# StellaOrg/ImplicitBVH.jl

Measured on AMD Instinct MI355X. Metric: BVH build+traverse throughput, higher is better.
Workload: dtype f32; 1 GPU; 1000000 random BSphere{Float32} leaves per GPU, BBox{Float32} nodes, UInt32 Morton, Int32 index, build + LVT self-traverse + read of the contact count (BASELINE.json configs[1]); leaves_per_gpu=1000000, leaves_total=1000000, contacts_total=1763579, parallelism=single GPU

## Files before the change

implicitbvh.jl_amd/csrc/ibvh_lvt_queue.inc:

```
#include "ibvh_lvt.hpp"

namespace ibvh {
namespace lvt {

#define IBVH_DPP_STEP(CTRL)                              \
    "v_min_f32_dpp %0, %0, %0 " CTRL "\n\t"              \
    "v_min_f32_dpp %1, %1, %1 " CTRL "\n\t"              \
    "v_min_f32_dpp %2, %2, %2 " CTRL "\n\t"              \
    "v_min_f32_dpp %3, %3, %3 " CTRL "\n\t"              \
    "v_min_f32_dpp %4, %4, %4 " CTRL "\n\t"              \
    "v_min_f32_dpp %5, %5, %5 " CTRL "\n\t"              \
    "v_max_f32_dpp %6, %6, %6 " CTRL "\n\t"              \
    "v_max_f32_dpp %7, %7, %7 " CTRL "\n\t"              \
    "v_max_f32_dpp %8, %8, %8 " CTRL "\n\t"              \
    "v_max_f32_dpp %9, %9, %9 " CTRL "\n\t"              \
    "v_max_f32_dpp %10, %10, %10 " CTRL "\n\t"           \
    "v_max_f32_dpp %11, %11, %11 " CTRL "\n\t"
IBVH_D void wave_prefix_scans_dpp(float (&mn)[6], float (&mx)[6]) {
    asm volatile("s_nop 1\n\t" IBVH_DPP_STEP("row_shr:1 row_mask:0xf bank_mask:0xf") IBVH_DPP_STEP("row_shr:2 row_mask:0xf bank_mask:0xf")
                     IBVH_DPP_STEP("row_shr:4 row_mask:0xf bank_mask:0xf") IBVH_DPP_STEP("row_shr:8 row_mask:0xf bank_mask:0xf")
                         IBVH_DPP_STEP("row_bcast:15 row_mask:0xa bank_mask:0xf") IBVH_DPP_STEP("row_bcast:31 row_mask:0xc bank_mask:0xf")
                 : "+v"(mn[0]), "+v"(mn[1]), "+v"(mn[2]), "+v"(mn[3]), "+v"(mn[4]), "+v"(mn[5]), "+v"(mx[0]), "+v"(mx[1]), "+v"(mx[2]),
                   "+v"(mx[3]), "+v"(mx[4]), "+v"(mx[5]));
}
#undef IBVH_DPP_STEP
IBVH_D float wave_min_dpp_lane63(float v) {
    asm volatile("s_nop 1\n\t"
                 "v_min_f32_dpp %0, %0, %0 row_shr:1 row_mask:0xf bank_mask:0xf\n\ts_nop 1\n\t"
                 "v_min_f32_dpp %0, %0, %0 row_shr:2 row_mask:0xf bank_mask:0xf\n\ts_nop 1\n\t"
                 "v_min_f32_dpp %0, %0, %0 row_shr:4 row_mask:0xf bank_mask:0xf\n\ts_nop 1\n\t"
                 "v_min_f32_dpp %0, %0, %0 row_shr:8 row_mask:0xf bank_mask:0xf\n\ts_nop 1\n\t"
                 "v_min_f32_dpp %0, %0, %0 row_bcast:15 row_mask:0xa bank_mask:0xf\n\ts_nop 1\n\t"
                 "v_min_f32_dpp %0, %0, %0 row_bcast:31 row_mask:0xc bank_mask:0xf\n\ts_nop 1"
                 : "+v"(v));
    return v;
}

#define IBVH_TEST_AND_APPEND(SFX, SEVENTH)                                                                                \
    asm volatile("s_mov_b64 exec, %[init]\n\t"                                                                           \
                 "v_cmpx_le" SFX " %[slo0], %[vup0]\n\t"                                                                 \
                 "v_cmpx_ge" SFX " %[sup0], %[vlo0]\n\t"                                                                 \
                 "v_cmpx_le" SFX " %[slo1], %[vup1]\n\t"                                                                 \
                 "v_cmpx_ge" SFX " %[sup1], %[vlo1]\n\t"                                                                 \
                 "v_cmpx_le" SFX " %[slo2], %[vup2]\n\t"                                                                 \
                 "v_cmpx_ge" SFX " %[sup2], %[vlo2]\n\t" SEVENTH "s_nop 2\n\t"                                          \
                 "v_mbcnt_lo_u32_b32 %[tmp], exec_lo, 0\n\t"                                                             \
                 "v_mbcnt_hi_u32_b32 %[tmp], exec_hi, %[tmp]\n\t"                                                        \
                 "v_lshl_add_u32 %[tmp], %[tmp], 2, %[addr]\n\t"                                                         \
                 "ds_write_b32 %[tmp], %[e]\n\t"                                                                         \
                 "s_bcnt1_i32_b64 %[cnt], exec\n\t"                                                                      \
                 "s_mov_b64 exec, -1\n\t"                                                                                \
                 "s_lshl2_add_u32 %[addr], %[cnt], %[addr]"                                                              \
                 : [tmp] "=&v"(tmp), [cnt] "=&s"(cnt), [addr] "+s"(lds_addr)                                             \
                 : [init] "s"(init), [slo0] "s"(slo0), [slo1] "s"(slo1), [slo2] "s"(slo2), [sup0] "s"(sup0), [sup1] "s"(sup1), \
                   [sup2] "s"(sup2), [vlo0] "v"(vlo0), [vlo1] "v"(vlo1), [vlo2] "v"(vlo2), [vup0] "v"(vup0), [vup1] "v"(vup1), \
                   [vup2] "v"(vup2), [sthr] "s"(sthr), [vcmp] "v"(vcmp), [e] "v"(e)                                      \
                 : "vcc", "scc", "memory")

#define IBVH_CONTACT_MASK(SFX)                                                                                                                \
    asm volatile("s_mov_b64 exec, %[init]\n\t"                                                                                               \
                 "v_cmpx_le" SFX " %[slo0], %[vup0]\n\t"                                                                                     \
                 "v_cmpx_ge" SFX " %[sup0], %[vlo0]\n\t"                                                                                     \
                 "v_cmpx_le" SFX " %[slo1], %[vup1]\n\t"                                                                                     \
                 "v_cmpx_ge" SFX " %[sup1], %[vlo1]\n\t"                                                                                     \
                 "v_cmpx_le" SFX " %[slo2], %[vup2]\n\t"                                                                                     \
                 "v_cmpx_ge" SFX " %[sup2], %[vlo2]\n\t"                                                                                     \
                 "s_mov_b64 %[m], exec\n\t"                                                                                                  \
                 "s_mov_b64 exec, -1"                                                                                                        \
                 : [m] "=&s"(m)                                                                                                              \
                 : [init] "s"(init), [slo0] "s"(S.lo[0]), [slo1] "s"(S.lo[1]), [slo2] "s"(S.lo[2]), [sup0] "s"(S.up[0]), [sup1] "s"(S.up[1]), \
                   [sup2] "s"(S.up[2]), [vlo0] "v"(V.lo[0]), [vlo1] "v"(V.lo[1]), [vlo2] "v"(V.lo[2]), [vup0] "v"(V.up[0]), [vup1] "v"(V.up[1]), \
                   [vup2] "v"(V.up[2])                                                                                                       \
                 : "vcc")

#define IBVH_CONTACT_MASK2(SFX)                                                                                                               \
    asm volatile("s_mov_b64 exec, %[init]\n\t"                                                                                               \
                 "v_cmpx_le" SFX " %[alo0], %[vup0]\n\t"                                                                                     \
                 "v_cmpx_ge" SFX " %[aup0], %[vlo0]\n\t"                                                                                     \
                 "v_cmpx_le" SFX " %[alo1], %[vup1]\n\t"                                                                                     \
                 "v_cmpx_ge" SFX " %[aup1], %[vlo1]\n\t"                                                                                     \
                 "v_cmpx_le" SFX " %[alo2], %[vup2]\n\t"                                                                                     \
                 "v_cmpx_ge" SFX " %[aup2], %[vlo2]\n\t"                                                                                     \
                 "s_mov_b64 %[ma], exec\n\t"                                                                                                 \
                 "s_mov_b64 exec, %[init]\n\t"                                                                                               \
                 "v_cmpx_le" SFX " %[blo0], %[vup0]\n\t"                                                                                     \
                 "v_cmpx_ge" SFX " %[bup0], %[vlo0]\n\t"                                                                                     \
                 "v_cmpx_le" SFX " %[blo1], %[vup1]\n\t"                                                                                     \
                 "v_cmpx_ge" SFX " %[bup1], %[vlo1]\n\t"                                                                                     \
                 "v_cmpx_le" SFX " %[blo2], %[vup2]\n\t"                                                                                     \
                 "v_cmpx_ge" SFX " %[bup2], %[vlo2]\n\t"                                                                                     \
                 "s_or_b64 %[m], %[ma], exec\n\t"                                                                                            \
                 "s_mov_b64 exec, -1"                                                                                                        \
                 : [m] "=&s"(m), [ma] "=&s"(ma)                                                                                              \
                 : [init] "s"(init), [alo0] "s"(A.lo[0]), [alo1] "s"(A.lo[1]), [alo2] "s"(A.lo[2]), [aup0] "s"(A.up[0]), [aup1] "s"(A.up[1]), \
                   [aup2] "s"(A.up[2]), [blo0] "s"(B.lo[0]), [blo1] "s"(B.lo[1]), [blo2] "s"(B.lo[2]), [bup0] "s"(B.up[0]), [bup1] "s"(B.up[1]), \
                   [bup2] "s"(B.up[2]), [vlo0] "v"(V.lo[0]), [vlo1] "v"(V.lo[1]), [vlo2] "v"(V.lo[2]), [vup0] "v"(V.up[0]), [vup1] "v"(V.up[1]), \
                   [vup2] "v"(V.up[2])                                                                                                       \
                 : "vcc", "scc")

#define IBVH_BOX_ASM(T, SFX)                                                                                                                  \
    template <bool THR_GE, bool PRUNE = true>                                                                                                \
    IBVH_D void test_and_append(uint64_t init, T slo0, T slo1, T slo2, T sup0, T sup1, T sup2, T vlo0, T vlo1, T vlo2, T vup0, T vup1, T vup2, \
                                uint32_t sthr, uint32_t vcmp, uint32_t e, uint32_t &lds_addr) {                                              \
        uint32_t tmp, cnt;                                                                                                                   \
        if constexpr (!PRUNE) IBVH_TEST_AND_APPEND(SFX, "");                                                                                 \
        else if constexpr (THR_GE) IBVH_TEST_AND_APPEND(SFX, "v_cmpx_ge_u32 %[sthr], %[vcmp]\n\t");                                          \
        else IBVH_TEST_AND_APPEND(SFX, "v_cmpx_lt_u32 %[sthr], %[vcmp]\n\t");                                                                \
    }                                                                                                                                        \
    IBVH_D uint64_t contact_mask(uint64_t init, const BBox<T> &S, const BBox<T> &V) {                                                        \
        uint64_t m;                                                                                                                          \
        IBVH_CONTACT_MASK(SFX);                                                                                                              \
        return m;                                                                                                                            \
    }                                                                                                                                        \
    IBVH_D uint64_t contact_mask2(uint64_t init, const BBox<T> &A, const BBox<T> &B, const BBox<T> &V) {                                     \
        uint64_t m, ma;                                                                                                                      \
        IBVH_CONTACT_MASK2(SFX);                                                                                                             \
        return m;                                                                                                                            \
    }
IBVH_BOX_ASM(float, "_f32")
IBVH_BOX_ASM(double, "_f64")
#undef IBVH_BOX_ASM
#undef IBVH_CONTACT_MASK2
#undef IBVH_CONTACT_MASK
#undef IBVH_TEST_AND_APPEND

IBVH_D void split_two_boxes_f32(const BBox<float> &mine, bool use, int lane, BBox<float> &ubox_a, BBox<float> &ubox_b) {
    using N = BBox<float>;
    const float big = float_max<float>();
    auto half_area = [](const N &b) {
        float d[3];
#pragma unroll
        for (int k = 0; k < 3; ++k) {
            d[k] = b.up[k] - b.lo[k];
            d[k] = d[k] > 0.0f ? d[k] : 0.0f;
        }
        return d[0] * d[1] + d[1] * d[2] + d[0] * d[2];
    };
    N pre, rev, rsuf;
#pragma unroll
    for (int k = 0; k < 3; ++k) {
        pre.lo[k] = use ? mine.lo[k] : big;
        pre.up[k] = use ? mine.up[k] : -big;
        rev.lo[k] = __shfl(pre.lo[k], 63 - lane, 64);
        rev.up[k] = __shfl(pre.up[k], 63 - lane, 64);
    }
    {
        float mn[6] = {pre.lo[0], pre.lo[1], pre.lo[2], rev.lo[0], rev.lo[1], rev.lo[2]};
        float mx[6] = {pre.up[0], pre.up[1], pre.up[2], rev.up[0], rev.up[1], rev.up[2]};
        wave_prefix_scans_dpp(mn, mx);
#pragma unroll
        for (int k = 0; k < 3; ++k) {
            pre.lo[k] = mn[k];
            pre.up[k] = mx[k];
            rsuf.lo[k] = mn[3 + k];
            rsuf.up[k] = mx[3 + k];
        }
    }
    const float ra = half_area(rsuf);
    float sa = __shfl(ra, 62 - lane, 64);
    sa = lane == 63 ? 0.0f : sa;
    float cost = half_area(pre) + sa;
    cost = cost == cost ? cost : __builtin_inff();
    const float m = wave_min_dpp_lane63(cost);
    const float best = __int_as_float(__builtin_amdgcn_readlane(__float_as_int(m), 63));
    const uint64_t at = __builtin_amdgcn_ballot_w64(cost == best);
    const int ksplit = at != 0 ? (int)__builtin_ctzll(at) : 0;
    ubox_a = broadcast_from_lane(pre, ksplit);
    ubox_b = broadcast_from_lane(rsuf, ksplit == 63 ? 0 : 62 - ksplit);
    if (ksplit == 63) {
#pragma unroll
        for (int k = 0; k < 3; ++k) {
            ubox_b.lo[k] = big;
            ubox_b.up[k] = -big;
        }
    }
}

template <class N> struct BlockFrontier {
    const N *nodes;
    TreeDev tree;
    const N *q_nodes;
    TreeDev q_tree;
    int32_t shift, start_level, cut_level, self;
    uint32_t *rows;
};
template <class N, bool PAIRED> __global__ __launch_bounds__(64) void lvt_block_frontier_kernel(BlockFrontier<N> f) {
    __shared__ uint32_t s_fr[2][BLK_FCAP];
    const int lane = threadIdx.x;
    const uint32_t b = blockIdx.x;
    uint32_t *row = f.rows + (size_t)b * BLK_ROW;
    const int levels = (int)f.tree.levels;
    const uint32_t vl = (uint32_t)f.tree.virtual_leaves;
    auto num_real = [&](int level) -> uint32_t { return (1u << (level - 1)) - (vl >> (levels - level)); };
    auto first_mem = [&](int level) -> uint32_t {
        const uint32_t v = vl >> (levels - (level - 1));
        return (1u << (level - 1)) - (2u * v - (uint32_t)__builtin_popcount(v)) - 1u;
    };
    const int qlevels = (int)f.q_tree.levels;
    const uint32_t qvl = (uint32_t)f.q_tree.virtual_leaves;
    const int blevel = qlevels - f.shift;
    const uint32_t qv = qvl >> (qlevels - (blevel - 1));
    const uint32_t q_first = (1u << (blevel - 1)) - (2u * qv - (uint32_t)__builtin_popcount(qv)) - 1u;
    const N bbox = load_vol_uniform<N>(f.q_nodes + (q_first + b));
    bool ok = true;
#pragma unroll
    for (int k = 0; k < 3; ++k) ok = ok && bbox.lo[k] == bbox.lo[k] && bbox.up[k] == bbox.up[k];
    if (lane == 0) *(N *)(row + 2) = bbox;
    if (!ok) {
        if (lane == 0) row[0] = 0xffffffffu;
        return;
    }
    const uint32_t block_next = (b << f.shift) + (1u << (levels - 1)) + 1u;
    const int start_level = f.start_level, cut_level = f.cut_level;
    auto touches = [&](const N &box, uint32_t idx, int lvl) {
        bool h = iscontact(bbox, box);
        if (f.self) h = h & !((idx + 1u) <= (block_next >> (levels - lvl)));
        return h;
    };
    int count = (int)num_real(start_level);
    for (int i = lane; i < count; i += 64) s_fr[0][i] = (1u << (start_level - 1)) + (uint32_t)i;
    __builtin_amdgcn_wave_barrier();
    uint32_t *cur = s_fr[0], *nxt = s_fr[1];
    const uint64_t lt_mask = ((uint64_t)1 << lane) - 1;
    int out = 0;
    bool overflow = false;
    int lvl = start_level;
    while (lvl <= cut_level && count > 0 && !overflow) {
        const N *lvl_nodes = f.nodes + first_mem(lvl);
        const uint32_t lvl_first = 1u << (lvl - 1);
        int next_count = 0;
        const bool paired = PAIRED && lvl < cut_level;
        if (paired) {
            const int cl = lvl + 1;
            const N *ch_nodes = f.nodes + first_mem(cl);
            const uint32_t ch_first = 1u << (cl - 1), ch_last = ch_first + num_real(cl) - 1u;
            const uint32_t gc_last = cl < levels ? (1u << cl) + num_real(cl + 1) - 1u : 0u;
            for (int base = 0; base < count; base += 64) {
                const bool have = base + lane < count;
                const uint32_t idx = cur[have ? base + lane : base];
                const uint32_t c0 = 2u * idx, c1 = c0 + 1u;
                const bool real1 = c1 <= ch_last;
                const N box = load_vol<N>(lvl_nodes + (idx - lvl_first));
                const N b0 = load_vol<N>(ch_nodes + (c0 - ch_first));
                const N b1 = load_vol<N>(ch_nodes + ((real1 ? c1 : c0) - ch_first));
                const bool hit = have & touches(box, idx, lvl);
                const bool h0 = hit & touches(b0, c0, cl), h1 = hit & real1 & touches(b1, c1, cl);
                const uint64_t m0 = __builtin_amdgcn_ballot_w64(h0), m1 = __builtin_amdgcn_ballot_w64(h1);
                const int before = __popcll(m0 & lt_mask) + __popcll(m1 & lt_mask), total = __popcll(m0) + __popcll(m1);
                if (cl == cut_level) {
                    if (out + total > BLK_CAP) {
                        overflow = true;
                        break;
                    }
                    if (h0) row[BLK_HEAD + out + before] = c0;
                    if (h1) row[BLK_HEAD + out + before + (h0 ? 1 : 0)] = c1;
                    out += total;
                } else {
                    if (next_count + 2 * total > BLK_FCAP) {
                        overflow = true;
                        break;
                    }
                    const int at = next_count + 2 * before;
                    if (h0) {
                        nxt[at] = 2u * c0;
                        nxt[at + 1] = 2u * c0 + 1u;
                    }
                    if (h1) {
                        nxt[at + (h0 ? 2 : 0)] = 2u * c1;
                        nxt[at + (h0 ? 2 : 0) + 1] = 2u * c1 + 1u;
                    }
                    const uint64_t any = m0 | m1;
                    bool last_virtual = false;
                    if (any != 0) {
                        const int top = 63 - __builtin_clzll(any);
                        const uint32_t ti = (uint32_t)__builtin_amdgcn_readlane((int)idx, top);
                        const uint32_t tc = ((m1 >> top) & 1u) ? 2u * ti + 1u : 2u * ti;
                        last_virtual = 2u * tc + 1u > gc_last;
                    }
                    next_count = __builtin_amdgcn_readfirstlane(next_count + 2 * total - (last_virtual ? 1 : 0));
                }
            }
            lvl += 2;
        } else {
            const uint32_t child_real = lvl < levels ? num_real(lvl + 1) : 0u;
            for (int base = 0; base < count; base += 64) {
                const bool have = base + lane < count;
                const uint32_t idx = cur[have ? base + lane : base];
                const N box = load_vol<N>(lvl_nodes + (idx - lvl_first));
                const bool hit = have & touches(box, idx, lvl);
                const uint64_t hm = __builtin_amdgcn_ballot_w64(hit);
                const int before = __popcll(hm & lt_mask), total = __popcll(hm);
                if (lvl == cut_level) {
                    if (out + total > BLK_CAP) {
                        overflow = true;
                        break;
                    }
                    if (hit) row[BLK_HEAD + out + before] = idx;
                    out += total;
                } else {
                    const bool last_virtual = hm != 0 && [&] {
                        const int top = 63 - __builtin_clzll(hm);
                        const uint32_t ti = (uint32_t)__builtin_amdgcn_readlane((int)idx, top);
                        return (2u * ti + 1u - (1u << lvl)) >= child_real;
                    }();
                    const int add = __builtin_amdgcn_readfirstlane(2 * total - (last_virtual ? 1 : 0));
                    if (next_count + add > BLK_FCAP) {
                        overflow = true;
                        break;
                    }
                    if (hit) {
                        nxt[next_count + 2 * before] = 2u * idx;
                        if (2 * before + 1 < add) nxt[next_count + 2 * before + 1] = 2u * idx + 1u;
                    }
                    next_count = __builtin_amdgcn_readfirstlane(next_count + add);
                }
            }
            lvl += 1;
        }
        __builtin_amdgcn_wave_barrier();
        uint32_t *t = cur;
        cur = nxt;
        nxt = t;
        count = __builtin_amdgcn_readfirstlane(lvl > cut_level ? 0 : next_count);
    }
    if (lane == 0) row[0] = overflow ? 0xffffffffu : (uint32_t)out;
}

#ifdef IBVH_PHASE_STAMPS
__device__ unsigned long long g_lvt_ticks[8];
struct Sections {
    unsigned long long t0, acc[6] = {0, 0, 0, 0, 0, 0};
    IBVH_D void start() { t0 = __builtin_amdgcn_s_memtime(); }
    IBVH_D void lap(int k) {
        const unsigned long long t = __builtin_amdgcn_s_memtime();
        acc[k] += t - t0;
        t0 = t;
    }
    IBVH_D void flush() {
        if ((threadIdx.x & 63) == 0) {
#pragma unroll
            for (int k = 0; k < 6; ++k) atomicAdd(&g_lvt_ticks[k], acc[k]);
            atomicAdd(&g_lvt_ticks[7], 1ull);
        }
    }
};
#else
struct Sections {
    IBVH_D void start() {}
    IBVH_D void lap(int) {}
    IBVH_D void flush() {}
};
#endif
enum { SEC_PROLOGUE = 0, SEC_DESCENT = 1, SEC_SUBTREE = 2, SEC_LOOPS = 3, SEC_LEAVES = 4, SEC_EPILOGUE = 5 };

constexpr int QUEUE_CAP = 512;
constexpr int QUEUE_WAVES = 1;
constexpr int QUEUE_MINWAVES = 7;

template <class L, class N, class I, bool WIDE, bool WRITE = false> constexpr int queue_min_waves() {
    if (sizeof(typename N::elt) == 8) return 4;
    if (sizeof(typename L::elt) == 8) return 5;
    if (WIDE && sizeof(I) == 8) return 6;
    return WRITE ? QUEUE_MINWAVES - 1 : QUEUE_MINWAVES;
}
template <class L, class N, class I, int MODE, bool WRITE, bool NARROW, bool WIDE, bool COUNT = false, class Q = L>
__global__ __launch_bounds__(64 * QUEUE_WAVES, (queue_min_waves<L, N, I, WIDE, WRITE>())) void lvt_queue_kernel(Args<L, N, I> a, PairCache<I> cache, int cut_level) {
    using TN = typename N::elt;
    static_assert(std::is_same<TN, float>::value || std::is_same<TN, double>::value,
                  "walker 2's box tests are assembly for Float32 and Float64 nodes (IBVH_BOX_ASM): a new node element type starts in dispatch_leaf_node");
    Work<COUNT> work;
    using QS = Query<L, N, I, MODE, WRITE, NARROW, Q>;
    using Cnt = typename QS::Cnt;
    __shared__ uint32_t s_frontier[QUEUE_WAVES][2][FRONTIER_CAP];
    using QE = typename std::conditional<WIDE, uint64_t, uint32_t>::type;
    __shared__ QE s_queue[QUEUE_WAVES][QUEUE_CAP];
    __shared__ Cnt s_cnt[QUEUE_WAVES][64];
    __shared__ I s_qside[QUEUE_WAVES][64];
    Sections sec;
    sec.start();
    const bool dense_index = WRITE && a.q_index_dense != nullptr;
    QS q(a, cache, dense_index);
    const int lane = threadIdx.x & 63, wv = __builtin_amdgcn_readfirstlane((int)(threadIdx.x >> 6));
    if constexpr (!WRITE && !COUNT) {
        if (a.q_index_dense != nullptr && q.valid) a.q_index_dense[q.item] = q.q_index;
        if (a.scan_agg != nullptr && lane == 0) {
            const int gw = (int)blockIdx.x * QUEUE_WAVES + wv;
            if (gw < a.scan_nparts) a.scan_agg[gw] = 0ull;
        }
    }
    struct Entry {
        I other;
        I meta;
    };
    const int64_t first_item = q.item - lane;
    const int64_t items_here = a.n_items - first_item < 64 ? a.n_items - first_item : 64;
    char *region = cache.K > 0 && items_here > 0 ? (char *)(cache.slots + first_item * (int64_t)cache.K) : nullptr;
    const int entry_cap = region ? (int)(((int64_t)items_here * cache.K * (int64_t)sizeof(IndexPair<I>) - 16) / (int64_t)sizeof(Entry)) : 0;
    Entry *entries = (Entry *)(region + 16);
    int wfill = 0;
    if constexpr (WRITE) {
        const int64_t guard = a.guard_total != nullptr ? load_total_uniform(a.guard_total) : 0;
        q.w = (q.valid && q.item > 0) ? (Cnt)a.counts[q.item - 1] : 0;
        const I q_side = a.positions ? (I)(q.item + 1) : ((dense_index && q.valid) ? a.q_index_dense[q.item] : q.q_index);
        const int fill_raw = region ? *(const int *)region : -1;
        constexpr bool SPECULATE = MODE == MODE_SELF;
        Entry e0 = {}, e1 = {};
        if constexpr (SPECULATE) {
            if (region && entry_cap > 0) {
                e0 = entries[lane < entry_cap ? lane : entry_cap - 1];
                e1 = entries[lane + 64 < entry_cap ? lane + 64 : entry_cap - 1];
            }
        }
        if (a.guard_total != nullptr && guard > a.guard_capacity) return;
        const int fill = __builtin_amdgcn_readfirstlane(fill_raw);
        if (fill >= 0) {
            s_cnt[wv][lane] = q.w;
            s_qside[wv][lane] = q_side;
            __builtin_amdgcn_wave_barrier();
            for (int t = lane; t < fill; t += 64) {
                const Entry e = !SPECULATE ? entries[t] : (t < 64 ? e0 : (t < 128 ? e1 : entries[t]));
                const int qi = (int)(e.meta & 63);
                const int64_t dest = (int64_t)s_cnt[wv][qi] + (int64_t)(e.meta >> 6);
                const I qv = s_qside[wv][qi];
                IndexPair<I> c2;
                if (a.positions) c2 = (MODE == MODE_PAIR && a.flip) ? IndexPair<I>{e.other, qv} : IndexPair<I>{qv, e.other};
                else if constexpr (MODE == MODE_SELF) c2 = qv > e.other ? IndexPair<I>{e.other, qv} : IndexPair<I>{qv, e.other};
                else c2 = a.flip ? IndexPair<I>{e.other, qv} : IndexPair<I>{qv, e.other};
                a.contacts[dest] = c2;
            }
            return;
        }
        if (dense_index) q.load_leaf();
        q.lane_on = q.valid;
    }
    if constexpr (MODE == MODE_PAIR) {
        if (a.built_level <= 1 && a.tree.levels >= 2) {
            const N root = load_vol_uniform<N>(a.nodes);
            work.add(0, q.lane_on);
            work.add(2, lane == 0);
            if (__builtin_amdgcn_ballot_w64(q.lane_on & iscontact(q.q_node, root)) == 0) {
                work.flush(a.work);
                if constexpr (!WRITE) {
                    if (q.valid) a.counts[q.item] = (I)0;
                    if (region && lane == 0) *(int *)region = 0;
                }
                return;
            }
        }
    }

    const int levels = (int)a.tree.levels;
    const uint32_t vl = (uint32_t)a.tree.virtual_leaves;
    auto num_real = [&](int level) -> uint32_t { return (1u << (level - 1)) - (vl >> (levels - level)); };
    auto first_mem = [&](int level) -> uint32_t {
        const uint32_t v = vl >> (levels - (level - 1));
        return (1u << (level - 1)) - (2u * v - (uint32_t)__builtin_popcount(v)) - 1u;
    };
    const uint32_t leaf_first = 1u << (levels - 1);
    const uint32_t my_item = (uint32_t)q.item;
    const uint32_t wave_item0 = (uint32_t)__builtin_amdgcn_readfirstlane((int)my_item);
    const uint32_t self_next = my_item + leaf_first + 1u;
    const uint32_t wave_next = wave_item0 + leaf_first + 1u;
    QE *queue = s_queue[wv];
    Cnt *cnts = s_cnt[wv];
    cnts[lane] = WRITE ? q.w : (Cnt)0;
    int qn = 0;
    const uint64_t lane_on_mask = __builtin_amdgcn_ballot_w64(q.lane_on);
    const uint32_t *blk_row = nullptr;
    int blk_count = -1;
    uint32_t blk_idx0 = 0;
    if constexpr (!COUNT) {
        if (a.blk_rows != nullptr) {
            blk_row = a.blk_rows + (size_t)(wave_item0 >> a.blk_shift) * BLK_ROW;
            blk_count = (int)*(const __attribute__((address_space(4))) uint32_t *)(uintptr_t)blk_row;
            blk_count = blk_count > BLK_CAP ? -1 : blk_count;
            blk_idx0 = blk_row[BLK_HEAD + lane];
        }
    }

    N ubox_a, ubox_b;
    {
        bool use = q.lane_on;
#pragma unroll
        for (int k = 0; k < 3; ++k) use = use && q.q_node.lo[k] == q.q_node.lo[k] && q.q_node.up[k] == q.q_node.up[k];
        if constexpr (std::is_same<TN, float>::value) {
            split_two_boxes_f32(q.q_node, use, lane, ubox_a, ubox_b);
        } else {
            BBox<float> qf, fa, fb;
#pragma unroll
            for (int k = 0; k < 3; ++k) {
                qf.lo[k] = __double2float_rd(q.q_node.lo[k]);
                qf.up[k] = __double2float_ru(q.q_node.up[k]);
            }
            split_two_boxes_f32(qf, use, lane, fa, fb);
#pragma unroll
            for (int k = 0; k < 3; ++k) {
                ubox_a.lo[k] = (double)fa.lo[k];
                ubox_a.up[k] = (double)fa.up[k];
                ubox_b.lo[k] = (double)fb.lo[k];
                ubox_b.up[k] = (double)fb.up[k];
            }
        }
    }
    bool use_rows = false;
    if constexpr (!COUNT) {
        if (blk_count >= 0) {
            const N bb = load_vol_uniform<N>(blk_row + 2);
            bool outside = false;
#pragma unroll
            for (int k = 0; k < 3; ++k) {
                const bool isnum = q.q_node.lo[k] == q.q_node.lo[k] && q.q_node.up[k] == q.q_node.up[k];
                outside = outside | (isnum & !(q.q_node.lo[k] >= bb.lo[k] && q.q_node.up[k] <= bb.up[k]));
            }
            bool allnum = true;
#pragma unroll
            for (int k = 0; k < 3; ++k) allnum = allnum && q.q_node.lo[k] == q.q_node.lo[k] && q.q_node.up[k] == q.q_node.up[k];
            use_rows = __builtin_amdgcn_ballot_w64(q.lane_on & allnum & outside) == 0;
        }
    }
    const int lp = levels - 1;
    const uint32_t lp_real = num_real(lp);
    const N *lp_nodes = a.nodes + first_mem(lp);
    const uint32_t n_leaves = (uint32_t)a.tree.real_leaves;
    const uint64_t lt_mask = ((uint64_t)1 << lane) - 1;

    auto pair_step = [&](int off, int avail) {
        const bool v = lane < avail;
        const QE e = queue[off + (v ? lane : 0)];
        const int qi = (int)(e & 63u);
        const uint32_t pos = 2u * (uint32_t)(e >> 6);
        const bool has_b = v & (pos + 1u < n_leaves);
        uint64_t mor_a = 0, mor_b = 0;
        const char *rec = a.leaves + (int64_t)pos * a.lay.stride;
        const char *rec_b = (pos + 1u < n_leaves) ? rec + a.lay.stride : rec;
        const L leaf_a = load_vol<L>(rec), leaf_b = load_vol<L>(rec_b);
        const I idx_a = load_index<I>(rec, a.lay), idx_b = load_index<I>(rec_b, a.lay);
        if constexpr (NARROW) {
            if (a.narrow == IBVH_NARROW_MORTON_LT) {
                mor_a = load_morton(rec, a.lay);
                mor_b = load_morton(rec_b, a.lay);
            }
        }
        const Q ql = shuffle_from(q.q_leaf, qi);
        const I qidx = __shfl(q.q_index, qi, 64);
        const uint32_t item_q = wave_item0 + (uint32_t)qi;
        bool hit_a = v & iscontact(ql, leaf_a), hit_b = has_b & iscontact(ql, leaf_b);
        work.add(1, (uint32_t)v + (uint32_t)has_b);
        work.add(3, (uint32_t)v + (uint32_t)has_b);
        if constexpr (MODE == MODE_SELF) {
            hit_a = hit_a & (pos > item_q);
            hit_b = hit_b & (pos + 1u > item_q);
        }
        if constexpr (NARROW) {
            const uint64_t qm = (uint64_t)__shfl((long long)q.q_morton, qi, 64);
            const bool fl = MODE == MODE_PAIR && a.flip;
            hit_a = hit_a && (fl ? narrow_eval(a.narrow, mor_a, idx_a, qm, qidx) : narrow_eval(a.narrow, qm, qidx, mor_a, idx_a));
            hit_b = hit_b && (fl ? narrow_eval(a.narrow, mor_b, idx_b, qm, qidx) : narrow_eval(a.narrow, qm, qidx, mor_b, idx_b));
        }
        uint32_t same_lo, same_hi;
        {
            const uint64_t vm = avail >= 64 ? ~(uint64_t)0 : (((uint64_t)1 << avail) - 1);
            same_lo = (uint32_t)vm;
            same_hi = (uint32_t)(vm >> 32);
        }
#pragma unroll
        for (int b = 0; b < 6; ++b) {
            const int x = (int)((uint32_t)qi << (31 - b)) >> 31;
            const uint64_t m = __builtin_amdgcn_ballot_w64(x != 0);
            same_lo = __builtin_amdgcn_bitop3_b32(same_lo, (uint32_t)m, (uint32_t)x, 0x90);
            same_hi = __builtin_amdgcn_bitop3_b32(same_hi, (uint32_t)(m >> 32), (uint32_t)x, 0x90);
        }
        const uint64_t m_a = __builtin_amdgcn_ballot_w64(hit_a), m_b = __builtin_amdgcn_ballot_w64(hit_b);
        const uint32_t sa_lo = same_lo & (uint32_t)m_a, sa_hi = same_hi & (uint32_t)(m_a >> 32);
        const uint32_t sb_lo = same_lo & (uint32_t)m_b, sb_hi = same_hi & (uint32_t)(m_b >> 32);
        const int rank = (int)__builtin_amdgcn_mbcnt_hi(sb_hi, __builtin_amdgcn_mbcnt_lo(sb_lo, __builtin_amdgcn_mbcnt_hi(sa_hi, __builtin_amdgcn_mbcnt_lo(sa_lo, 0u))));
        const int tot = __builtin_popcount(sa_lo) + __builtin_popcount(sa_hi) + __builtin_popcount(sb_lo) + __builtin_popcount(sb_hi);
        const bool group_first = __builtin_amdgcn_mbcnt_hi(same_hi, __builtin_amdgcn_mbcnt_lo(same_lo, 0u)) == 0u;
        const Cnt base = cnts[qi];
        __builtin_amdgcn_wave_barrier();
        if (v && group_first && tot > 0) cnts[qi] = base + (Cnt)tot;
        __builtin_amdgcn_wave_barrier();
        auto put = [&](Cnt at, I lidx, int slot, uint32_t lpos) {
            if constexpr (WRITE) {
                IndexPair<I> c2;
                if (a.positions) {
                    const I qp = (I)(item_q + 1u), lp = (I)(lpos + 1u);
                    c2 = (MODE == MODE_PAIR && a.flip) ? IndexPair<I>{lp, qp} : IndexPair<I>{qp, lp};
                } else if constexpr (MODE == MODE_SELF) c2 = qidx > lidx ? IndexPair<I>{lidx, qidx} : IndexPair<I>{qidx, lidx};
                else c2 = a.flip ? IndexPair<I>{lidx, qidx} : IndexPair<I>{qidx, lidx};
                a.contacts[(int64_t)at] = c2;
            } else {
                if (slot < entry_cap) entries[slot] = Entry{a.positions ? (I)(lpos + 1u) : lidx, (I)((I)qi | ((I)(at - 0) << 6))};
            }
        };
        const Cnt at = base + (Cnt)rank;
        const int n_a = __popcll(m_a);
        auto below = [](uint64_t m) { return (int)__builtin_amdgcn_mbcnt_hi((uint32_t)(m >> 32), __builtin_amdgcn_mbcnt_lo((uint32_t)m, 0u)); };
        if (hit_a) put(at, idx_a, wfill + below(m_a), pos);
        if (hit_b) put(at + (hit_a ? 1 : 0), idx_b, wfill + n_a + below(m_b), pos + 1u);
        if constexpr (!WRITE) wfill = __builtin_amdgcn_readfirstlane(wfill + n_a + __popcll(m_b));
    };
    auto drain = [&](bool all) {
        sec.lap(SEC_LOOPS);
        int done = 0;
        while (qn - done >= 64 || (all && qn - done > 0)) {
            const int avail = qn - done < 64 ? qn - done : 64;
            pair_step(done, avail);
            done += avail;
        }
        const int rem = qn - done;
        if (rem > 0 && done > 0) {
            const QE e = lane < rem ? queue[done + lane] : (QE)0;
            __builtin_amdgcn_wave_barrier();
            if (lane < rem) queue[lane] = e;
            __builtin_amdgcn_wave_barrier();
        }
        qn = __builtin_amdgcn_readfirstlane(rem);
        sec.lap(SEC_LEAVES);
    };

    auto brute = [&](uint32_t c, const N &cbox) {
        sec.lap(SEC_DESCENT);
        work.add(0, q.lane_on);
        uint64_t on_mask;
        bool on;
        {
            uint64_t init = lane_on_mask;
            if constexpr (MODE == MODE_SELF) init &= __builtin_amdgcn_ballot_w64(!((c + 1u) <= (self_next >> (levels - cut_level))));
            on_mask = contact_mask(init, cbox, q.q_node);
            on = (on_mask >> lane) & 1u;
        }
        if (on_mask == 0) {
            sec.lap(SEC_SUBTREE);
            return;
        }
        const uint32_t first32 = (c - (1u << (cut_level - 1))) << (lp - cut_level);
        uint32_t last = first32 + (1u << (lp - cut_level));
        last = last < lp_real ? last : lp_real;
        const int np = (int)(last - first32);
        const N mybox = load_vol<N>(lp_nodes + (first32 + (uint32_t)(lane < np ? lane : np - 1)));
        const bool mine = lane < np;
        work.add(2, lane < np);
        work.add(0, lane < np ? 2u : 0u);
        const uint32_t right_leaf = 2u * (first32 + (uint32_t)lane) + 1u;
        uint64_t box_mask;
        bool box_on;
        {
            uint64_t init = __builtin_amdgcn_ballot_w64(mine);
            if constexpr (MODE == MODE_SELF) init &= __builtin_amdgcn_ballot_w64(right_leaf > wave_item0);
            box_mask = contact_mask2(init, ubox_a, ubox_b, mybox);
            box_on = (box_mask >> lane) & 1u;
        }
        uint32_t n_box = (uint32_t)__builtin_popcountll(box_mask), n_on = (uint32_t)__builtin_popcountll(on_mask);
        asm volatile("" : "+s"(n_box), "+s"(n_on));
        const bool by_box = n_box < n_on;
        sec.lap(SEC_SUBTREE);
        const QE e_box = (QE)lane | ((QE)first32 << 6);
        const QE e_qry = (QE)(first32 + (uint32_t)lane) << 6;
        if constexpr (!WIDE) {
            const uint32_t queue_lds = (uint32_t)(uintptr_t)(__attribute__((address_space(3))) uint32_t *)queue;
            const uint32_t drain_at = queue_lds + 4u * (uint32_t)(QUEUE_CAP - 64);
            uint32_t qaddr = queue_lds + 4u * (uint32_t)qn;
            auto drain_if_full = [&]() {
                if (qaddr > drain_at) {
                    qn = (int)((qaddr - queue_lds) >> 2);
                    drain(false);
                    qaddr = queue_lds + 4u * (uint32_t)qn;
                }
            };
            const uint32_t half_item = MODE == MODE_SELF ? (my_item + 1u) >> 1 : 0u;
            auto loop_by_box = [&](auto prune) {
                for (uint64_t todo = box_mask; todo != 0;) {
                    drain_if_full();
                    const int u = __builtin_ctzll(todo);
                    asm("s_bitset0_b64 %0, %1" : "+s"(todo) : "s"(u));
                    const uint32_t pidx = first32 + (uint32_t)u;
                    const N p = load_vol_uniform<N>((const char *)lp_nodes + pidx * (uint32_t)sizeof(N));
                    work.add(0, (uint32_t)(on_mask >> lane) & 1u);
                    work.add(2, lane == 0);
                    test_and_append<true, decltype(prune)::value>(on_mask, p.lo[0], p.lo[1], p.lo[2], p.up[0], p.up[1], p.up[2], q.q_node.lo[0], q.q_node.lo[1],
                                              q.q_node.lo[2], q.q_node.up[0], q.q_node.up[1], q.q_node.up[2], pidx, half_item,
                                              e_box + ((uint32_t)u << 6), qaddr);
                }
            };
            auto loop_by_query = [&](auto prune) {
                for (uint64_t todo = on_mask; todo != 0;) {
                    drain_if_full();
                    const int u = __builtin_ctzll(todo);
                    asm("s_bitset0_b64 %0, %1" : "+s"(todo) : "s"(u));
                    const N qb = broadcast_from_lane(q.q_node, u);
                    work.add(0, (uint32_t)(box_mask >> lane) & 1u);
                    const uint32_t thr = MODE == MODE_SELF ? wave_item0 + (uint32_t)u : 0u;
                    test_and_append<false, decltype(prune)::value>(box_mask, qb.lo[0], qb.lo[1], qb.lo[2], qb.up[0], qb.up[1], qb.up[2], mybox.lo[0], mybox.lo[1],
                                               mybox.lo[2], mybox.up[0], mybox.up[1], mybox.up[2], thr, MODE == MODE_SELF ? right_leaf : 1u,
                                               e_qry | (uint32_t)u, qaddr);
                }
            };
            using Prune = std::integral_constant<bool, MODE == MODE_SELF>;
            if (by_box) loop_by_box(Prune{});
            else loop_by_query(Prune{});
            qn = (int)((qaddr - queue_lds) >> 2);
        } else {
            for (uint64_t todo = by_box ? box_mask : on_mask; todo != 0; todo &= todo - 1) {
                if (qn > QUEUE_CAP - 64) drain(false);
                const int u = __builtin_ctzll(todo);
                bool h;
                QE e;
                work.add(0, (uint32_t)((by_box ? on_mask : box_mask) >> lane) & 1u);
                if (by_box) {
                    const N pbox = broadcast_from_lane(mybox, u);
                    h = on & iscontact(q.q_node, pbox);
                    if constexpr (MODE == MODE_SELF) h = h & (2u * (first32 + (uint32_t)u) + 1u > my_item);
                    e = e_box + ((QE)u << 6);
                } else {
                    const N qbox = broadcast_from_lane(q.q_node, u);
                    h = box_on & iscontact(qbox, mybox);
                    if constexpr (MODE == MODE_SELF) h = h & (right_leaf > wave_item0 + (uint32_t)u);
                    e = e_qry | (QE)u;
                }
                const uint64_t hm = __builtin_amdgcn_ballot_w64(h);
                const int rank = (int)__builtin_amdgcn_mbcnt_hi((uint32_t)(hm >> 32), __builtin_amdgcn_mbcnt_lo((uint32_t)hm, 0u));
                if (h) queue[qn + rank] = e;
                qn = __builtin_amdgcn_readfirstlane(qn + __popcll(hm));
            }
        }
        sec.lap(SEC_LOOPS);
    };

    sec.lap(SEC_PROLOGUE);
    if (use_rows) {
        const N *cut_nodes = a.nodes + first_mem(cut_level);
        const uint32_t cut_first = 1u << (cut_level - 1), cut_real = num_real(cut_level);
        for (int base = 0; base < blk_count; base += 64) {
            const int at = base + lane < BLK_CAP ? base + lane : BLK_CAP - 1;
            uint32_t idx = base == 0 ? blk_idx0 : blk_row[BLK_HEAD + at];
            const bool have = (base + lane < blk_count) & (idx - cut_first < cut_real);
            idx = have ? idx : cut_first;
            const N box = load_vol<N>(cut_nodes + (idx - cut_first));
            uint64_t hit_mask;
            {
                bool pre = have;
                if constexpr (MODE == MODE_SELF) pre = pre & !((idx + 1u) <= (wave_next >> (levels - cut_level)));
                hit_mask = contact_mask2(__builtin_amdgcn_ballot_w64(pre), ubox_a, ubox_b, box);
            }
            for (uint64_t todo = hit_mask; todo != 0; todo &= todo - 1) {
                const int src = __builtin_ctzll(todo);
                const uint32_t c = (uint32_t)__builtin_amdgcn_readlane((int)idx, src);
                const N cbox = load_vol_uniform<N>((const char *)cut_nodes + (c - cut_first) * (uint32_t)sizeof(N));
                brute(c, cbox);
            }
        }
    } else {
    uint32_t *fr0 = s_frontier[wv][0], *fr1 = s_frontier[wv][1];
    const int start_level = (int)a.start_level;
    const uint32_t root_first = 1u << (start_level - 1);
    const int roots = (int)num_real(start_level);
    bool overflow = false;
    for (int r0 = 0; r0 < roots && !overflow; r0 += FRONTIER_CAP) {
        int count = __builtin_amdgcn_readfirstlane((roots - r0) < FRONTIER_CAP ? (roots - r0) : FRONTIER_CAP);
        for (int i = lane; i < count; i += 64) fr0[i] = root_first + (uint32_t)(r0 + i);
        __builtin_amdgcn_wave_barrier();
        uint32_t *cur = fr0, *nxt = fr1;
        for (int lvl = start_level; lvl <= cut_level && count > 0; ++lvl) {
            const N *lvl_nodes = a.nodes + first_mem(lvl);
            const uint32_t lvl_first = 1u << (lvl - 1);
            const uint32_t child_real = num_real(lvl + 1);
            int next_count = 0;
            for (int base = 0; base < count; base += 64) {
                const bool have = base + lane < count;
                work.add(2, have);
                work.add(0, have ? 2u : 0u);
                const uint32_t idx = cur[have ? base + lane : base];
                const N box = load_vol<N>(lvl_nodes + (idx - lvl_first));
                bool hit;
                uint64_t hit_mask;
                {
                    bool pre = have;
                    if constexpr (MODE == MODE_SELF) pre = pre & !((idx + 1u) <= (wave_next >> (levels - lvl)));
                    const uint64_t init = __builtin_amdgcn_ballot_w64(pre);
                    hit_mask = contact_mask2(init, ubox_a, ubox_b, box);
                    hit = (hit_mask >> lane) & 1u;
                }
                const uint64_t hm = hit_mask;
                if (lvl == cut_level) {
                    for (uint64_t todo = hm; todo != 0; todo &= todo - 1) {
                        const int src = __builtin_ctzll(todo);
                        const uint32_t c = (uint32_t)__builtin_amdgcn_readlane((int)idx, src);
                        const N cbox = load_vol_uniform<N>((const char *)lvl_nodes + (c - lvl_first) * (uint32_t)sizeof(N));
                        brute(c, cbox);
                    }
                } else {
                    const int before = __popcll(hm & lt_mask);
                    const int total = __popcll(hm);
                    const bool last_virtual = hm != 0 && [&] {
                        const int top = 63 - __builtin_clzll(hm);
                        const uint32_t ti = (uint32_t)__builtin_amdgcn_readlane((int)idx, top);
                        return (2u * ti + 1u - (1u << lvl)) >= child_real;
                    }();
                    const int add = __builtin_amdgcn_readfirstlane(2 * total - (last_virtual ? 1 : 0));
                    if (next_count + add > FRONTIER_CAP) {
                        overflow = true;
                        break;
                    }
                    if (hit) {
                        nxt[next_count + 2 * before] = 2u * idx;
                        if (2 * before + 1 < add) nxt[next_count + 2 * before + 1] = 2u * idx + 1u;
                    }
                    next_count = __builtin_amdgcn_readfirstlane(next_count + add);
                }
            }
            if (overflow) break;
            __builtin_amdgcn_wave_barrier();
            uint32_t *t = cur;
            cur = nxt;
            nxt = t;
            count = __builtin_amdgcn_readfirstlane(lvl == cut_level ? 0 : next_count);
        }
    }
    if (overflow) {
        q.cnt = 0;
        q.cache.K = 0;
        if constexpr (WRITE) q.w = (q.valid && q.item > 0) ? (Cnt)a.counts[q.item - 1] : 0;
        joint_walk(q, a);
        q.finish();
        work.flush(a.work);
        if constexpr (!WRITE)
            if (region && lane == 0) *(int *)region = -1;
        return;
    }
    }
    sec.lap(SEC_DESCENT);
    drain(true);
    work.flush(a.work);
    if constexpr (!WRITE) {
        if (q.valid) a.counts[q.item] = (I)cnts[lane];
        const bool meta_ok = __builtin_amdgcn_ballot_w64((int64_t)cnts[lane] >= ((int64_t)1 << (sizeof(I) * 8 - 7))) == 0;
        if (region && lane == 0) *(int *)region = (wfill <= entry_cap && meta_ok) ? wfill : -1;
    }
    sec.lap(SEC_EPILOGUE);
    sec.flush();
}

template <class L, class N, class I, int MODE, class Q>
int launch_queue(const Args<L, N, I> &a, const PairCache<I> &cache, bool write, hipStream_t st, bool *agg_zeroed) {
    static_assert(N::kind == IBVH_BBOX, "walker 2 needs nested node boxes");
    const bool count_work = a.work != nullptr;
    const bool force_wide = g_tuning.lvt_wide != 0;
    if (a.tree.levels > 31 || !(a.start_level < a.tree.levels)) return IBVH_ERR_UNSUPPORTED;
    const bool wide = force_wide || a.tree.levels > 28;
    Args<L, N, I> aq = a;
    aq.xcd_tiles = a.xcd_tiles > 1 ? a.xcd_tiles * 4 / QUEUE_WAVES : a.xcd_tiles;
    const unsigned qblocks = (unsigned)ceil_div(a.n_items, (int64_t)64 * QUEUE_WAVES);
    int64_t top = a.built_level > 7 ? a.built_level : 7;
    if (top > a.tree.levels - 1) top = a.tree.levels - 1;
    aq.start_level = top;
    const int64_t c = aq.tree.levels - BRUTE_DEPTH;
    const int cut = (int)(c > aq.start_level ? c : aq.start_level);
    if constexpr (kWorkTypes<L, N, I> && std::is_same<Q, L>::value) {
        if (count_work) {
            if (wide || aq.narrow != IBVH_NARROW_NONE) return IBVH_ERR_UNSUPPORTED;
            IBVH_LAUNCH((lvt_queue_kernel<L, N, I, MODE, false, false, false, true>), dim3(qblocks), dim3(64 * QUEUE_WAVES), 0, st,
                        aq, cache, cut);
            IBVH_LAUNCH_CHECK();
            return IBVH_OK;
        }
    }
    aq.blk_rows = nullptr;
    if (a.blk_rows != nullptr && g_tuning.lvt_blocks != 0) {
        const int shift = g_tuning.lvt_block_shift >= BLK_SHIFT_MIN && g_tuning.lvt_block_shift <= 12 ? g_tuning.lvt_block_shift : 11;
        const int64_t blevel = a.q_tree.levels - shift;
        const int64_t min_items = g_tuning.lvt_blocks_min_items > 0 ? g_tuning.lvt_blocks_min_items : (int64_t)1 << 17;
        if (blevel >= 1 && blevel >= a.q_built_level && cut - aq.start_level >= 2 && a.n_items >= min_items &&
            level_num_real(aq.tree.levels, aq.tree.virtual_leaves, aq.start_level) <= BLK_FCAP && a.tree.levels <= 28 && a.q_tree.levels <= 31) {
            if (!write) {
                BlockFrontier<N> f;
                f.nodes = aq.nodes, f.tree = aq.tree, f.q_nodes = a.q_nodes, f.q_tree = a.q_tree;
                f.shift = shift, f.start_level = (int)aq.start_level, f.cut_level = cut, f.self = MODE == MODE_SELF ? 1 : 0;
                f.rows = a.blk_rows;
                const unsigned nblk = (unsigned)ceil_div(a.n_items, (int64_t)1 << shift);
                const int paired_below = g_tuning.lvt_blocks_paired_below >= 0 ? g_tuning.lvt_blocks_paired_below : 4096;
                if ((int64_t)nblk < paired_below) IBVH_LAUNCH((lvt_block_frontier_kernel<N, true>), dim3(nblk), dim3(64), 0, st, f);
                else IBVH_LAUNCH((lvt_block_frontier_kernel<N, false>), dim3(nblk), dim3(64), 0, st, f);
            }
            aq.blk_rows = a.blk_rows;
            aq.blk_shift = shift;
        }
    }
    if (agg_zeroed) *agg_zeroed = !write && aq.scan_agg != nullptr;
    const int variant = (write ? 1 : 0) | (aq.narrow != IBVH_NARROW_NONE ? 2 : 0) | (wide ? 4 : 0);
#define IBVH_QUEUE_LAUNCH(W_, N_, D_)                                                                                 \
    IBVH_LAUNCH((lvt_queue_kernel<L, N, I, MODE, W_, N_, D_, false, Q>), dim3(qblocks), dim3(64 * QUEUE_WAVES), 0, st, aq, cache, cut)
    switch (variant) {
    case 0: IBVH_QUEUE_LAUNCH(false, false, false); break;
    case 1: IBVH_QUEUE_LAUNCH(true, false, false); break;
    case 2: IBVH_QUEUE_LAUNCH(false, true, false); break;
    case 3: IBVH_QUEUE_LAUNCH(true, true, false); break;
    case 4: IBVH_QUEUE_LAUNCH(false, false, true); break;
    case 5: IBVH_QUEUE_LAUNCH(true, false, true); break;
    case 6: IBVH_QUEUE_LAUNCH(false, true, true); break;
    default: IBVH_QUEUE_LAUNCH(true, true, true); break;
    }
#undef IBVH_QUEUE_LAUNCH
    IBVH_LAUNCH_CHECK();
    return IBVH_OK;
}

#define IBVH_INSTANTIATE_QUEUE(L_, N_, I_, MODE_) \
    template int launch_queue<L_, N_, I_, MODE_, L_>(const Args<L_, N_, I_> &, const PairCache<I_> &, bool, hipStream_t, bool *);

}
}
```

Measured before the change: 4547 Mleaves/s.

## Move same-query rank computation from count pass to replay pass

In the count (non-write) pass, per-query hit counts are now bumped with wave-scope LDS atomics and entries store only the query lane, instead of running the six-ballot same-query ranking per pair step. The ranking is moved into the cached-entry replay path, where each 64-entry chunk recomputes destinations against the shared counters. This drops the meta overflow check, because the rank is no longer packed into entry metadata. The count pass gets cheaper while the write replay does more work, and correctness now relies on entry order matching the per-query rank order.

```diff
diff --git a/implicitbvh.jl_amd/csrc/ibvh_lvt_queue.inc b/implicitbvh.jl_amd/csrc/ibvh_lvt_queue.inc
--- a/implicitbvh.jl_amd/csrc/ibvh_lvt_queue.inc
+++ b/implicitbvh.jl_amd/csrc/ibvh_lvt_queue.inc
@@ -353,6 +353,27 @@
 #endif
 enum { SEC_PROLOGUE = 0, SEC_DESCENT = 1, SEC_SUBTREE = 2, SEC_LOOPS = 3, SEC_LEAVES = 4, SEC_EPILOGUE = 5 };
 
+template <class Cnt> IBVH_D Cnt rank_same_query(Cnt *cnts, int qi, bool v, uint64_t vm, uint64_t m_a, uint64_t m_b) {
+    uint32_t same_lo = (uint32_t)vm, same_hi = (uint32_t)(vm >> 32);
+#pragma unroll
+    for (int b = 0; b < 6; ++b) {
+        const int x = (int)((uint32_t)qi << (31 - b)) >> 31;
+        const uint64_t m = __builtin_amdgcn_ballot_w64(x != 0);
+        same_lo = __builtin_amdgcn_bitop3_b32(same_lo, (uint32_t)m, (uint32_t)x, 0x90);
+        same_hi = __builtin_amdgcn_bitop3_b32(same_hi, (uint32_t)(m >> 32), (uint32_t)x, 0x90);
+    }
+    const uint32_t sa_lo = same_lo & (uint32_t)m_a, sa_hi = same_hi & (uint32_t)(m_a >> 32);
+    const uint32_t sb_lo = same_lo & (uint32_t)m_b, sb_hi = same_hi & (uint32_t)(m_b >> 32);
+    const int rank = (int)__builtin_amdgcn_mbcnt_hi(sb_hi, __builtin_amdgcn_mbcnt_lo(sb_lo, __builtin_amdgcn_mbcnt_hi(sa_hi, __builtin_amdgcn_mbcnt_lo(sa_lo, 0u))));
+    const int tot = __builtin_popcount(sa_lo) + __builtin_popcount(sa_hi) + __builtin_popcount(sb_lo) + __builtin_popcount(sb_hi);
+    const bool group_first = __builtin_amdgcn_mbcnt_hi(same_hi, __builtin_amdgcn_mbcnt_lo(same_lo, 0u)) == 0u;
+    const Cnt base = cnts[qi];
+    __builtin_amdgcn_wave_barrier();
+    if (v && group_first && tot > 0) cnts[qi] = base + (Cnt)tot;
+    __builtin_amdgcn_wave_barrier();
+    return base + (Cnt)rank;
+}
+
 constexpr int QUEUE_CAP = 512;
 constexpr int QUEUE_WAVES = 1;
 constexpr int QUEUE_MINWAVES = 7;
@@ -417,16 +438,20 @@
             s_cnt[wv][lane] = q.w;
             s_qside[wv][lane] = q_side;
             __builtin_amdgcn_wave_barrier();
-            for (int t = lane; t < fill; t += 64) {
-                const Entry e = !SPECULATE ? entries[t] : (t < 64 ? e0 : (t < 128 ? e1 : entries[t]));
+            for (int t0 = 0; t0 < fill; t0 += 64) {
+                const int left = fill - t0;
+                const bool v = lane < left;
+                const int t = t0 + (v ? lane : left - 1);
+                const Entry e = !SPECULATE ? entries[t] : (t0 == 0 ? e0 : (t0 == 64 ? e1 : entries[t]));
                 const int qi = (int)(e.meta & 63);
-                const int64_t dest = (int64_t)s_cnt[wv][qi] + (int64_t)(e.meta >> 6);
+                const uint64_t vm = left >= 64 ? ~(uint64_t)0 : (((uint64_t)1 << left) - 1);
+                const int64_t dest = (int64_t)rank_same_query(s_cnt[wv], qi, v, vm, vm, (uint64_t)0);
                 const I qv = s_qside[wv][qi];
                 IndexPair<I> c2;
                 if (a.positions) c2 = (MODE == MODE_PAIR && a.flip) ? IndexPair<I>{e.other, qv} : IndexPair<I>{qv, e.other};
                 else if constexpr (MODE == MODE_SELF) c2 = qv > e.other ? IndexPair<I>{e.other, qv} : IndexPair<I>{qv, e.other};
                 else c2 = a.flip ? IndexPair<I>{e.other, qv} : IndexPair<I>{qv, e.other};
-                a.contacts[dest] = c2;
+                if (v) a.contacts[dest] = c2;
             }
             return;
         }
@@ -557,48 +582,30 @@
             hit_a = hit_a && (fl ? narrow_eval(a.narrow, mor_a, idx_a, qm, qidx) : narrow_eval(a.narrow, qm, qidx, mor_a, idx_a));
             hit_b = hit_b && (fl ? narrow_eval(a.narrow, mor_b, idx_b, qm, qidx) : narrow_eval(a.narrow, qm, qidx, mor_b, idx_b));
         }
-        uint32_t same_lo, same_hi;
-        {
+        const uint64_t m_a = __builtin_amdgcn_ballot_w64(hit_a), m_b = __builtin_amdgcn_ballot_w64(hit_b);
+        auto below = [](uint64_t m) { return (int)__builtin_amdgcn_mbcnt_hi((uint32_t)(m >> 32), __builtin_amdgcn_mbcnt_lo((uint32_t)m, 0u)); };
+        if constexpr (WRITE) {
             const uint64_t vm = avail >= 64 ? ~(uint64_t)0 : (((uint64_t)1 << avail) - 1);
-            same_lo = (uint32_t)vm;
-            same_hi = (uint32_t)(vm >> 32);
-        }
-#pragma unroll
-        for (int b = 0; b < 6; ++b) {
-            const int x = (int)((uint32_t)qi << (31 - b)) >> 31;
-            const uint64_t m = __builtin_amdgcn_ballot_w64(x != 0);
-            same_lo = __builtin_amdgcn_bitop3_b32(same_lo, (uint32_t)m, (uint32_t)x, 0x90);
-            same_hi = __builtin_amdgcn_bitop3_b32(same_hi, (uint32_t)(m >> 32), (uint32_t)x, 0x90);
-        }
-        const uint64_t m_a = __builtin_amdgcn_ballot_w64(hit_a), m_b = __builtin_amdgcn_ballot_w64(hit_b);
-        const uint32_t sa_lo = same_lo & (uint32_t)m_a, sa_hi = same_hi & (uint32_t)(m_a >> 32);
-        const uint32_t sb_lo = same_lo & (uint32_t)m_b, sb_hi = same_hi & (uint32_t)(m_b >> 32);
-        const int rank = (int)__builtin_amdgcn_mbcnt_hi(sb_hi, __builtin_amdgcn_mbcnt_lo(sb_lo, __builtin_amdgcn_mbcnt_hi(sa_hi, __builtin_amdgcn_mbcnt_lo(sa_lo, 0u))));
-        const int tot = __builtin_popcount(sa_lo) + __builtin_popcount(sa_hi) + __builtin_popcount(sb_lo) + __builtin_popcount(sb_hi);
-        const bool group_first = __builtin_amdgcn_mbcnt_hi(same_hi, __builtin_amdgcn_mbcnt_lo(same_lo, 0u)) == 0u;
-        const Cnt base = cnts[qi];
-        __builtin_amdgcn_wave_barrier();
-        if (v && group_first && tot > 0) cnts[qi] = base + (Cnt)tot;
-        __builtin_amdgcn_wave_barrier();
-        auto put = [&](Cnt at, I lidx, int slot, uint32_t lpos) {
-            if constexpr (WRITE) {
+            const Cnt at = rank_same_query(cnts, qi, v, vm, m_a, m_b);
+            auto put = [&](Cnt to, I lidx, uint32_t lpos) {
                 IndexPair<I> c2;
                 if (a.positions) {
                     const I qp = (I)(item_q + 1u), lp = (I)(lpos + 1u);
                     c2 = (MODE == MODE_PAIR && a.flip) ? IndexPair<I>{lp, qp} : IndexPair<I>{qp, lp};
                 } else if constexpr (MODE == MODE_SELF) c2 = qidx > lidx ? IndexPair<I>{lidx, qidx} : IndexPair<I>{qidx, lidx};
                 else c2 = a.flip ? IndexPair<I>{lidx, qidx} : IndexPair<I>{qidx, lidx};
-                a.contacts[(int64_t)at] = c2;
-            } else {
-                if (slot < entry_cap) entries[slot] = Entry{a.positions ? (I)(lpos + 1u) : lidx, (I)((I)qi | ((I)(at - 0) << 6))};
-            }
-        };
-        const Cnt at = base + (Cnt)rank;
-        const int n_a = __popcll(m_a);
-        auto below = [](uint64_t m) { return (int)__builtin_amdgcn_mbcnt_hi((uint32_t)(m >> 32), __builtin_amdgcn_mbcnt_lo((uint32_t)m, 0u)); };
-        if (hit_a) put(at, idx_a, wfill + below(m_a), pos);
-        if (hit_b) put(at + (hit_a ? 1 : 0), idx_b, wfill + n_a + below(m_b), pos + 1u);
-        if constexpr (!WRITE) wfill = __builtin_amdgcn_readfirstlane(wfill + n_a + __popcll(m_b));
+                a.contacts[(int64_t)to] = c2;
+            };
+            if (hit_a) put(at, idx_a, pos);
+            if (hit_b) put(at + (hit_a ? 1 : 0), idx_b, pos + 1u);
+        } else {
+            const uint32_t hits = (uint32_t)hit_a + (uint32_t)hit_b;
+            if (hits != 0) __hip_atomic_fetch_add(&cnts[qi], (Cnt)hits, __ATOMIC_RELAXED, __HIP_MEMORY_SCOPE_WAVEFRONT);
+            const int slot_a = wfill + below(m_a) + below(m_b), slot_b = slot_a + (hit_a ? 1 : 0);
+            if (hit_a && slot_a < entry_cap) entries[slot_a] = Entry{a.positions ? (I)(pos + 1u) : idx_a, (I)qi};
+            if (hit_b && slot_b < entry_cap) entries[slot_b] = Entry{a.positions ? (I)(pos + 2u) : idx_b, (I)qi};
+            wfill = __builtin_amdgcn_readfirstlane(wfill + __popcll(m_a) + __popcll(m_b));
+        }
     };
     auto drain = [&](bool all) {
         sec.lap(SEC_LOOPS);
@@ -833,9 +840,9 @@
     drain(true);
     work.flush(a.work);
     if constexpr (!WRITE) {
+        __builtin_amdgcn_wave_barrier();
         if (q.valid) a.counts[q.item] = (I)cnts[lane];
-        const bool meta_ok = __builtin_amdgcn_ballot_w64((int64_t)cnts[lane] >= ((int64_t)1 << (sizeof(I) * 8 - 7))) == 0;
-        if (region && lane == 0) *(int *)region = (wfill <= entry_cap && meta_ok) ? wfill : -1;
+        if (region && lane == 0) *(int *)region = wfill <= entry_cap ? wfill : -1;
     }
     sec.lap(SEC_EPILOGUE);
     sec.flush();
```

New measurement: 4645 Mleaves/s (median of 6 runs). 1.02x the previous value.
